# hku-mars/FAST_LIO

Hardware: NVIDIA H100
Metric: scans/sec (30k-pt scan, 1M-pt map iEKF) (higher is better)
Workload: dtype f32 geometry / f64 filter

## Files before the change

### fast_lio_b200/api.py

```python
from __future__ import annotations

import ctypes as C
import os

import numpy as np

from . import build as _build

_f32p = np.ctypeslib.ndpointer(dtype=np.float32, flags="C_CONTIGUOUS")
_f64p = np.ctypeslib.ndpointer(dtype=np.float64, flags="C_CONTIGUOUS")
_i32p = np.ctypeslib.ndpointer(dtype=np.int32, flags="C_CONTIGUOUS")
_u8p = np.ctypeslib.ndpointer(dtype=np.uint8, flags="C_CONTIGUOUS")


class PassLog(C.Structure):
    _fields_ = [("searched", C.c_int), ("valid", C.c_int), ("effct", C.c_int), ("converged", C.c_int),
                ("res_sum", C.c_double), ("HtH", C.c_double * 144), ("Hth", C.c_double * 12),
                ("x_after", C.c_double * 26)]


def _log_dict(l: PassLog) -> dict:
    return dict(searched=l.searched, valid=l.valid, effct=l.effct, converged=l.converged,
                res_sum=l.res_sum, HtH=np.array(l.HtH).reshape(12, 12).copy(),
                Hth=np.array(l.Hth).copy(), x_after=np.array(l.x_after).copy())
# ... 15 lines not shown

LIDAR_AVIA, LIDAR_VELO16, LIDAR_OUST64, LIDAR_MARSIM = 1, 2, 3, 4
TIME_SEC, TIME_MS, TIME_US, TIME_NS = 0, 1, 2, 3
CUSTOM_POINT = np.dtype({"names": ["offset_time", "x", "y", "z", "reflectivity", "tag", "line"],
                         "formats": ["<u4", "<f4", "<f4", "<f4", "u1", "u1", "u1"],
                         "offsets": [0, 4, 8, 12, 16, 17, 18], "itemsize": 20})
VELODYNE_POINT = np.dtype({"names": ["x", "y", "z", "intensity", "time", "ring"],
                           "formats": ["<f4", "<f4", "<f4", "<f4", "<f4", "<u2"],
                           "offsets": [0, 4, 8, 16, 20, 24], "itemsize": 32})
OUSTER_POINT = np.dtype({"names": ["x", "y", "z", "intensity", "t", "reflectivity", "ring", "ambient", "range"],
                         "formats": ["<f4", "<f4", "<f4", "<f4", "<u4", "<u2", "u1", "<u2", "<u4"],
                         "offsets": [0, 4, 8, 16, 20, 24, 26, 28, 32], "itemsize": 48})
POINT_XYZI = np.dtype({"names": ["x", "y", "z", "intensity"], "formats": ["<f4"] * 4, "offsets": [0, 4, 8, 16], "itemsize": 32})
DEFAULT_LAYOUT = {LIDAR_AVIA: CUSTOM_POINT, LIDAR_VELO16: VELODYNE_POINT, LIDAR_OUST64: OUSTER_POINT, LIDAR_MARSIM: POINT_XYZI}
OFFSET_FIELDS = ("x", "y", "z", "intensity", "time", "ring", "tag", "line")
_FIELD_NAMES = {LIDAR_AVIA: {"intensity": "reflectivity", "time": "offset_time"}, LIDAR_OUST64: {"time": "t"}}


def layout_offsets(dtype: np.dtype, lidar_type: int) -> list[int]:
    names = _FIELD_NAMES.get(lidar_type, {})
    fields = dtype.fields or {}
    return [int(fields[names.get(f, f)][1]) if names.get(f, f) in fields else -1 for f in OFFSET_FIELDS]


class PreprocessParams(C.Structure):
    _fields_ = [("lidar_type", C.c_int), ("n_scans", C.c_int), ("scan_rate", C.c_int), ("time_unit", C.c_int),
                ("point_filter_num", C.c_int), ("blind", C.c_double), ("point_step", C.c_int)] + \
               [("off_" + f, C.c_int) for f in OFFSET_FIELDS]


_lib = None

SYMBOLS = [
    "fl_last_error", "fl_device_count", "fl_version", "fl_host_register", "fl_host_unregister", "fl_filter_debug_prof",
    "fl_map_create", "fl_map_destroy", "fl_map_set_downsample", "fl_map_build", "fl_map_size", "fl_map_validnum",
    "fl_map_knn", "fl_map_nearest_search", "fl_map_add_points", "fl_map_delete_boxes", "fl_map_flatten", "fl_map_tree_range",
    "fl_map_rebuild", "fl_map_stats", "fl_map_add_boxes", "fl_map_box_search", "fl_map_radius_search", "fl_map_acquire_removed", "fl_map_set_cell_directory", "fl_map_dir_stats",
    "fl_map_set_deterministic", "fl_map_get_deterministic",
    "fl_map_nearest_search_device", "fl_map_range_workspace_bytes", "fl_map_box_search_device", "fl_map_radius_search_device",
    "fl_map_build_device", "fl_map_add_points_device",
    "fl_filter_create", "fl_filter_destroy", "fl_filter_set_params", "fl_filter_set_solver", "fl_filter_set_search", "fl_filter_set_fused", "fl_filter_update",
    "fl_filter_map_incremental", "fl_filter_get_nearest", "fl_filter_get_selected", "fl_filter_get_pass_logs", "fl_filter_upload_scan",
    "fl_filter_upload_state", "fl_filter_run", "fl_filter_download_state", "fl_filter_sync",
    "fl_filter_time_resident", "fl_filter_time_search_pass", "fl_filter_time_e2e", "fl_filter_gpu_launches",
    "fl_scan_create", "fl_scan_destroy", "fl_scan_upload", "fl_scan_undistort", "fl_scan_voxel_downsample", "fl_scan_download",
    "fl_filter_update_scan", "fl_localmap_create", "fl_localmap_destroy", "fl_localmap_segment", "fl_localmap_get",
    "fl_comm_unique_id", "fl_filter_comm_init", "fl_filter_set_shard", "fl_filter_p2p_handle", "fl_filter_p2p_connect",
    "fl_filter_update_device", "fl_filter_get_nearest_device", "fl_filter_get_selected_device",
    "fl_map_add_points_async", "fl_map_maintain", "fl_filter_map_incremental_device",
    "fl_scan_reserve", "fl_scan_upload_device", "fl_scan_undistort_device", "fl_scan_voxel_downsample_device",
    "fl_filter_update_scan_device", "fl_map_delete_boxes_async", "fl_localmap_segment_device",
    "fl_filter_reserve_batch", "fl_filter_batch_plan", "fl_filter_update_batch_device",
    "fl_preprocess_create", "fl_preprocess_destroy", "fl_preprocess_device", "fl_preprocess",
    "fl_scan_frame", "fl_scan_frame_device",
]


def lib_path() -> str:
    return _build.LIB


def load():
    global _lib
    if _lib is not None:
        return _lib
    if not os.path.exists(_build.LIB):
        raise FastLioError(f"{_build.LIB} is missing -- run `python -m fast_lio_b200.build` (nvcc, sm_90a); "
# ... 801 lines not shown
```

### fast_lio_b200/build.py

```python
from __future__ import annotations

import os
import shutil
import subprocess
import sys

HERE = os.path.dirname(os.path.abspath(__file__))
CSRC = os.path.join(HERE, "csrc")
LIB = os.path.join(HERE, "libfastlio_b200.so")
SOURCES = ["map.cu", "filter.cu", "scan.cu", "preprocess.cu", "capi.cu"]
HEADERS = ["common.cuh", "map.cuh", "map.h", "lie.cuh", "filter.h", "scan.h", "gj.cuh", "measure.cuh", "update.cuh", "upd_plan.h", "preprocess.h", os.path.join("..", "..", "include", "fastlio_b200.h")]

NVCC_FLAGS = [
    "-gencode", "arch=compute_90a,code=sm_90a",
    "-O3", "-std=c++17", "-lineinfo",
    "--fmad=false", "-prec-div=true", "-prec-sqrt=true",
    "-Xcompiler", "-fPIC", "-shared",
    "-Xptxas", "-v",
]


def _nvcc() -> str:
    for cand in (os.environ.get("NVCC"), "/usr/local/cuda/bin/nvcc", shutil.which("nvcc")):
        if cand and os.path.exists(cand):
            return cand
    raise RuntimeError("nvcc not found")


def needs_build() -> bool:
    if not os.path.exists(LIB):
        return True
    t = os.path.getmtime(LIB)
    deps = [os.path.join(CSRC, s) for s in SOURCES + HEADERS] + [os.path.abspath(__file__)]
    return any(os.path.getmtime(d) > t for d in deps if os.path.exists(d))


def build(force: bool = False, verbose: bool = False) -> str:
    if not force and not needs_build():
        return LIB
    tmp = LIB + ".tmp"
    cmd = [_nvcc()] + NVCC_FLAGS + ["-ccbin", "/usr/bin/g++"] + [os.path.join(CSRC, s) for s in SOURCES] + ["-o", tmp, "-ldl"]
    res = subprocess.run(cmd, capture_output=True, text=True)
    log = res.stdout + res.stderr
    with open(os.path.join(HERE, "build.log"), "w") as f:
        f.write(" ".join(cmd) + "\n" + log)
    if res.returncode != 0:
        sys.stderr.write(log)
        raise RuntimeError("nvcc failed")
    os.replace(tmp, LIB)
    if verbose:
        print(log)
    return LIB


if __name__ == "__main__":
    build(force="--force" in sys.argv, verbose=True)
```

### fast_lio_b200/csrc/capi.cu

```cuda
#include <atomic>
#include <chrono>
#include <cstring>
#include <mutex>
#include <new>

#include "../../include/fastlio_b200.h"
#include "filter.h"
#include "preprocess.h"
#include "scan.h"

namespace fl {
const char* last_error();
int nccl_unique_id(void* out128);
}

struct fl_map {
    fl::Map* impl;
    std::mutex mu;
    std::atomic<int> refs{1};
};
static void map_retain(fl_map* m) { m->refs.fetch_add(1, std::memory_order_relaxed); }
static void map_release(fl_map* m) {
    if (m->refs.fetch_sub(1, std::memory_order_acq_rel) == 1) {
        delete m->impl;
// ... 281 lines not shown
    FILTER_GUARD(f);
    if (!out3) { fl::set_last_error("fl_filter_batch_plan: null out3"); return FL_ERR_ARG; }
    return f->impl->batch_plan(nq, n_hyp, &out3[0], &out3[1], &out3[2]);
}
int fl_filter_update_batch_device(fl_filter_t* f, const float* body_xyzi_device, int nq, int n_hyp, double* x26_device, double* P_device,
                                  double R, int* status2_device, fl_pass_log_t* logs_device, void* stream) {
    FILTER_GUARD(f);
    return f->impl->update_batch_on_stream(body_xyzi_device, nq, n_hyp, x26_device, P_device, R, status2_device,
                                           reinterpret_cast<fl::PassLog*>(logs_device), static_cast<cudaStream_t>(stream));
}
int fl_filter_get_nearest_device(fl_filter_t* f, float* out_pts_device, int* out_cnt_device, int nq, void* stream) {
    FILTER_GUARD(f);
    return f->impl->get_nearest_on_stream(out_pts_device, out_cnt_device, nq, static_cast<cudaStream_t>(stream));
}
int fl_filter_get_selected_device(fl_filter_t* f, unsigned char* out_device, int nq, void* stream) {
    FILTER_GUARD(f);
    return f->impl->get_selected_on_stream(out_device, nq, static_cast<cudaStream_t>(stream));
}
int fl_filter_upload_scan(fl_filter_t* f, const float* body, int nq) { FILTER_GUARD(f); return f->impl->upload_scan(body, nq); }
int fl_filter_upload_state(fl_filter_t* f, const double* x26, const double* P, double R) {
    FILTER_GUARD(f);
    if (!x26 || !P) return FL_ERR_ARG;
    return f->impl->upload_state(x26, P, R);
}
int fl_filter_run(fl_filter_t* f) { FILTER_HOST_GUARD(f); return f->impl->run_passes(); }
int fl_filter_download_state(fl_filter_t* f, double* x26, double* P, int* n_pass) { FILTER_GUARD(f); return f->impl->download_state(x26, P, n_pass); }
int fl_filter_sync(fl_filter_t* f) { FILTER_GUARD(f); return f->impl->sync(); }
int fl_filter_debug_prof(fl_filter_t* f, long long* out16) {
    FILTER_GUARD(f);
    if (!out16) return FL_ERR_ARG;
    FL_CUDA(cudaMemcpy(out16, f->impl->ctl_device()->prof, sizeof(long long) * 16, cudaMemcpyDeviceToHost));
    for (int i = 0; i < 4; i++) out16[12 + i] = f->impl->host_ns()[i];
    return FL_OK;
}
int fl_filter_gpu_launches(fl_filter_t* f) { FILTER_GUARD(f); return f->impl->gpu_launches(); }

int fl_filter_time_resident(fl_filter_t* f, int reps, int flush_l2, float* ms_total) {
    FILTER_GUARD(f);
    if (reps < 1 || !ms_total) return FL_ERR_ARG;
    fl::Filter* F = f->impl;
    cudaStream_t st = F->stream();
    FL_CUDA(cudaSetDevice(F->map()->device()));
    const size_t flush_bytes = 256u << 20;
    if (flush_l2) FL_CHECK(f->flush.reserve(flush_bytes));
    cudaEvent_t e0, e1;
    FL_CUDA(cudaEventCreate(&e0));
    FL_CUDA(cudaEventCreate(&e1));
    float total = 0.f;
    for (int r = 0; r < reps; r++) {
        FL_CHECK(F->restore_state());
        if (flush_l2) FL_CUDA(cudaMemsetAsync(f->flush.ptr, r & 0xff, flush_bytes, st));
        FL_CHECK(F->p2p_barrier());
        FL_CUDA(cudaEventRecord(e0, st));
        int rc = F->run_passes();
        if (rc != FL_OK) { cudaEventDestroy(e0); cudaEventDestroy(e1); return rc; }
        FL_CUDA(cudaEventRecord(e1, st));
        FL_CUDA(cudaEventSynchronize(e1));
        float ms = 0.f;
        FL_CUDA(cudaEventElapsedTime(&ms, e0, e1));
        total += ms;
    }
    cudaEventDestroy(e0);
    cudaEventDestroy(e1);
    *ms_total = total;
    return FL_OK;
}
// ... 283 lines not shown
```

### fast_lio_b200/csrc/filter.cu

```cuda
#include <dlfcn.h>

#include <algorithm>
#include <chrono>
#include <cstdlib>

#include <cub/device/device_select.cuh>

#include "filter.h"
#include "gj.cuh"
#include "measure.cuh"

namespace fl {

constexpr int PSTRIDE = 96;
constexpr size_t P2P_MAIL_BYTES = sizeof(unsigned long long) * 2 * 2 * P2P_MAX_RANKS * PSTRIDE;
constexpr int SEARCH_THREADS = 256;
constexpr int SEARCH_C_THREADS = 256;
constexpr int RESID_THREADS = 256;
constexpr int MAX_LOGS = 16;

__device__ __forceinline__ void pdl_wait() { asm volatile("griddepcontrol.wait;" ::: "memory"); }
__device__ __forceinline__ void pdl_launch() { asm volatile("griddepcontrol.launch_dependents;" ::: "memory"); }

__device__ __forceinline__ int tri12(int a, int b) { return a * 12 - (a * (a - 1)) / 2 + (b - a); }
// ... 984 lines not shown
    if (nq < 0 || (nq > 0 && !body_xyzi)) { set_last_error("scan: bad arguments"); return FL_ERR_ARG; }
    FL_CUDA(cudaSetDevice(map_->device()));
    FL_CHECK(reserve(std::max(1, nq)));
    if (nq > 0) FL_CUDA(cudaMemcpyAsync(body_.ptr, body_xyzi, sizeof(float4) * (size_t)nq, cudaMemcpyHostToDevice, stream()));
    return set_scan_device(body_.as<float4>(), nq);
}

int Filter::set_shard(int q_begin, int q_end) {
    if (q_begin < 0 || q_end < q_begin) { set_last_error("set_shard: bad range"); return FL_ERR_ARG; }
    scan_.q_begin = q_begin; scan_.q_end = q_end;
    shard_set_ = true;
    return FL_OK;
}

int Filter::upload_state(const double* x26, const double* P, double R, bool snapshot) {
    FL_CUDA(cudaSetDevice(map_->device()));
    FL_CUDA(cudaStreamSynchronize(stream()));
    FilterCtl& c = *h_ctl_;
    c.iter = -1; c.t = 0; c.converge = 1; c.done = 0; c.n_pass = 0; c.error = 0; c.ticket = 0; c.gen = 0;
    c.max_iter = max_iter_;
    c.host_mirror = (mirror_ && !snapshot) ? h_ctl_ : nullptr;
    c.extrinsic_est = extrinsic_est_;
    c.R = R;
    for (int i = 0; i < NDOF; i++) c.limit[i] = limit_[i];
    memcpy(c.x, x26, sizeof(double) * XLEN);
    memcpy(c.x_prop, x26, sizeof(double) * XLEN);
    memcpy(c.P, P, sizeof(double) * NDOF * NDOF);
    memcpy(c.P_prop, P, sizeof(double) * NDOF * NDOF);
    FL_CUDA(cudaMemcpyAsync(ctl_.ptr, h_ctl_, sizeof(FilterCtl), cudaMemcpyHostToDevice, stream()));
    if (snapshot) FL_CUDA(cudaMemcpyAsync(ctl0_.ptr, ctl_.ptr, sizeof(FilterCtl), cudaMemcpyDeviceToDevice, stream()));
    return FL_OK;
}

int Filter::restore_state() {
    FL_CUDA(cudaSetDevice(map_->device()));
    FL_CUDA(cudaMemcpyAsync(ctl_.ptr, ctl0_.ptr, sizeof(FilterCtl), cudaMemcpyDeviceToDevice, stream()));
    return FL_OK;
}

template <class... KArgs, class... Args>
static cudaError_t launch_pdl_smem(void (*kernel)(KArgs...), dim3 grid, int block, size_t smem, cudaStream_t st, bool pdl, Args... args) {
    cudaLaunchConfig_t cfg;
    memset(&cfg, 0, sizeof(cfg));
    cfg.gridDim = grid; cfg.blockDim = dim3((unsigned)block); cfg.dynamicSmemBytes = smem; cfg.stream = st;
    cudaLaunchAttribute attr[1];
    attr[0].id = cudaLaunchAttributeProgrammaticStreamSerialization;
    attr[0].val.programmaticStreamSerializationAllowed = pdl ? 1 : 0;
    cfg.attrs = attr; cfg.numAttrs = 1;
    return cudaLaunchKernelEx(&cfg, kernel, KArgs(args)...);
}
template <class... KArgs, class... Args>
static cudaError_t launch_pdl(void (*kernel)(KArgs...), dim3 grid, int block, cudaStream_t st, bool pdl, Args... args) {
    return launch_pdl_smem(kernel, grid, block, 0, st, pdl, args...);
}

int Filter::complete_neighbours() {
    if (neighbours_complete_ || (scan_.q_begin <= 0 && scan_.q_end >= scan_.Q)) { neighbours_complete_ = true; return FL_OK; }
    FL_CUDA(cudaSetDevice(map_->device()));
    const int keep_b = scan_.q_begin, keep_e = scan_.q_end;
    const int ranges[2][2] = {{0, keep_b}, {keep_e, scan_.Q}};
    for (int r = 0; r < 2; r++) {
        if (ranges[r][1] <= ranges[r][0]) continue;
        scan_.q_begin = ranges[r][0]; scan_.q_end = ranges[r][1];
        UpdArgs a = upd_args(1, 0, 1);
        a.dbg = 0; a.pose_from_search = 1;
        cudaError_t e = launch_plan(plan(UR_NEIGHBOURS, scan_.q_end - scan_.q_begin), a, stream());
// ... 626 lines not shown
```

### fast_lio_b200/csrc/filter.h

```cpp
#pragma once
#include "lie.cuh"
#include "map.h"
#include "upd_plan.h"

namespace fl {

struct PassLog {
    int searched, valid, effct, converged;
    double res_sum;
    double HtH[144];
    double Hth[12];
    double x_after[XLEN];
};

struct FilterCtl {
    int iter;
    int t;
    int converge;
    int done;
    int n_pass;
    int max_iter;
    int extrinsic_est;
    int error;
    int ticket;
// ... 57 lines not shown
    int download_state(double* x26, double* P, int* n_pass);
    int sync();
    int update_on_stream(const float* d_body, int nq, double* d_x26, double* d_P, double R, int* d_status2, cudaStream_t st);
    int get_nearest_on_stream(float* d_pts, int* d_cnt, int nq, cudaStream_t st);
    int get_selected_on_stream(unsigned char* d_out, int nq, cudaStream_t st);
    int update_scan_on_stream(const float4* d_body, const int* d_n, int n_max, double* d_x26, double* d_P, double R, int* d_status2, cudaStream_t st);
    int capacity() const;
    int reserve_batch(int nq_max);
    int batch_plan(int nq, int n_hyp, int* workers, int* slots, int* waves) const;
    int update_batch_on_stream(const float* d_body, int nq, int n_hyp, double* d_x26, double* d_P, double R, int* d_status2,
                               PassLog* d_logs, cudaStream_t st);

    int map_incremental(double filter_size_map_min, int ekf_inited, int* n_to_add, int* n_no_downsample, int* added);
    int map_incremental_on_stream(double filter_size_map_min, int ekf_inited, int* d_out4, cudaStream_t st);
    int get_nearest(float* out_pts, int* out_cnt, int nq);
    int complete_neighbours();
    int get_selected(unsigned char* out, int nq);
    int get_pass_logs(PassLog* out, int cap, int* n);
    int comm_init(int nranks, int rank, const void* nccl_unique_id_128);
    int set_shard(int q_begin, int q_end);
    int p2p_local_handle(void* out64);
    int p2p_connect(int nranks, int rank, const void* handles64);
    int p2p_barrier();

    void set_fused(bool on) { fused_ = on; }
    bool fused() const { return fused_ && solver_ == 1; }
    int gpu_launches() const { return launches_; }
    const long long* host_ns() const { return host_ns_; }
    const float4* nearest_device() const { return scan_.nearest; }
    const ScanView& scan() const { return scan_; }
    cudaStream_t stream() const { return map_->stream(); }
    Map* map() const { return map_; }
    const FilterCtl* ctl_device() const { return ctl_.as<FilterCtl>(); }

private:
    int reserve(int nq);
    int update_any(const float* body_xyzi, const float4* d_body, int nq, double* x26, double* P, double R, double* solve_time_s);
    Map* map_;
    int max_points_;
    int max_iter_ = 4;
    double limit_[NDOF];
    int extrinsic_est_ = 0;
    int solver_ = 1;
    bool mirror_ = true;
    bool pdl_ = true;
    int search_occ_ = 5;
    int search_mode_ = 1;
    ScanView scan_;
    DeviceBuffer srange_;
    DeviceBuffer body_, nearest_, nearest_cnt_, selected_, normvec_, plane_, partials_, red_, ctl_, ctl0_, logs_;
    DeviceBuffer mi_world_, mi_flag_add_, mi_flag_no_, mi_list_add_, mi_list_no_, mi_tmp_, mi_counts_;
    FilterCtl* h_ctl_ = nullptr;
    cudaEvent_t ev0_ = nullptr, ev1_ = nullptr;
    int sms_ = 0, search_grid_max_ = 0, max_resid_grid_ = 0, resid_grid_ = 1;
    bool fused_ = true;
    DeviceBuffer pub_;
    unsigned launch_nonce_ = 0;
    UpdCaps upd_caps_ = {};
    int launch_update(int max_passes, int mode, int search_only) { return launch_update(max_passes, mode, search_only, stream()); }
    int launch_update(int max_passes, int mode, int search_only, cudaStream_t st);
    UpdPlan plan(UpdRoute r, int rows, int n_hyp = 0) const;
    cudaError_t launch_plan(const UpdPlan& p, const UpdArgs& a, cudaStream_t st, const int* n = nullptr, int log_stride = 0);
    StateIn state_in_args(double R) const;
    int device_form_scope(const char* what, bool update) const;
    UpdArgs upd_args(int max_passes, int mode, int search_only);
    int bind_scan(const float4* d_body, int nq);
// ... 23 lines not shown
```

### fast_lio_b200/csrc/update.cuh

```cuda
#pragma once

namespace fl {

constexpr int UPD_THREADS = 256;
constexpr int UPD_WARPS = UPD_THREADS / 32;

struct UpdArgs {
    MapView m;
    ScanView sc;
    FilterCtl* ctl;
    double* partials;
    double* red_g;
    PassLog* logs;
    P2PState* p2p;
    unsigned long long* pub;
    unsigned nonce;
    int mode;
    int max_passes;
    int search_only;
    int dbg;
    int pose_from_search;
};

struct SolverSm {
// ... 21 lines not shown
    WalkPool walks;
    unsigned pose_bits[28];
    unsigned flags;
    int abort;
};

__device__ __forceinline__ int ld_acquire(const int* p) {
    int v;
    asm volatile("ld.acquire.gpu.global.s32 %0, [%1];" : "=r"(v) : "l"(p) : "memory");
    return v;
}
__device__ __forceinline__ void st_release(int* p, int v) { asm volatile("st.release.gpu.global.s32 [%0], %1;" ::"l"(p), "r"(v) : "memory"); }
constexpr long long SPIN_LIMIT = 3000000000ll;

constexpr int PUB_WORDS = 29;
__device__ __forceinline__ unsigned pub_tag(unsigned nonce, int pass) { return (nonce << 8) | (unsigned)(pass & 0xff); }
__device__ __forceinline__ void pub_store(unsigned long long* p, unsigned tag, unsigned payload) {
    asm volatile("st.relaxed.gpu.global.u64 [%0], %1;" ::"l"(p), "l"(((unsigned long long)tag << 32) | payload) : "memory");
}
__device__ __forceinline__ unsigned long long pub_load(const unsigned long long* p) {
    unsigned long long v;
    asm volatile("ld.relaxed.gpu.global.u64 %0, [%1];" : "=l"(v) : "l"(p) : "memory");
    return v;
}
__device__ __forceinline__ void pub_publish(unsigned long long* pub, unsigned tag, const double* x, int converge, int done, int lane) {
    if (lane < 28) {
        const unsigned long long bits = (unsigned long long)__double_as_longlong(x[lane >> 1]);
        pub_store(pub + lane, tag, (lane & 1) ? (unsigned)(bits >> 32) : (unsigned)bits);
    } else if (lane == 28) {
        pub_store(pub + 28, tag, (converge ? 1u : 0u) | (done ? 2u : 0u));
    }
}


template <bool DET>
__device__ __forceinline__ void cell_scan_chunks(const MapView& m, int start, int cnt, int c0, int c1, float qx, float qy, float qz, TBestT<DET>& kb) {
    const int4* list = reinterpret_cast<const int4*>(m.dir.lists + start);
    int4 ia = make_int4(0, 0, 0, 0), ib = make_int4(0, 0, 0, 0);
    if (c0 < c1) {
        ia = __ldg(&list[2 * c0]);
        if (cnt - 8 * c0 > 4) ib = __ldg(&list[2 * c0 + 1]);
    }
#pragma unroll 1
    for (int c = c0; c < c1; c++) {
        const int n8 = cnt - 8 * c;
        float4 p0, p1, p2, p3, p4, p5, p6, p7;
        p1 = p2 = p3 = p4 = p5 = p6 = p7 = make_float4(0.f, 0.f, 0.f, 0.f);
        p0 = __ldg(&m.pts[ia.x]);
        if (n8 > 1) p1 = __ldg(&m.pts[ia.y]);
        if (n8 > 2) p2 = __ldg(&m.pts[ia.z]);
        if (n8 > 3) p3 = __ldg(&m.pts[ia.w]);
        if (n8 > 4) p4 = __ldg(&m.pts[ib.x]);
        if (n8 > 5) p5 = __ldg(&m.pts[ib.y]);
        if (n8 > 6) p6 = __ldg(&m.pts[ib.z]);
        if (n8 > 7) p7 = __ldg(&m.pts[ib.w]);
        int4 na = ia, nb = ib;
        if (c + 1 < c1) {
            na = __ldg(&list[2 * c + 2]);
            if (n8 > 12) nb = __ldg(&list[2 * c + 3]);
        }
        cell_consider(m, p0, ia.x, qx, qy, qz, kb);
        cell_consider(m, p1, ia.y, qx, qy, qz, kb);
        cell_consider(m, p2, ia.z, qx, qy, qz, kb);
        cell_consider(m, p3, ia.w, qx, qy, qz, kb);
        cell_consider(m, p4, ib.x, qx, qy, qz, kb);
        cell_consider(m, p5, ib.y, qx, qy, qz, kb);
// ... 42 lines not shown
        }
    }
    PairXch& X = *reinterpret_cast<PairXch*>(stage);
    pair_sync(warp);
    if (!owner) {
#pragma unroll
        for (int j = 0; j < KNN_K; j++) { X.d[j][lane] = kb.d[j]; X.idx[j][lane] = kb.idx[j]; }
    }
    pair_sync(warp);
    bool exact = true;
    if (owner && active) {
        exact = false;
        if (listed) {
            pair_merge(m, X, lane, kb);
            if (kb.idx[KNN_K - 1] >= 0) {
                const float g = cell_block_dist(D, qx, qy, qz, ix, iy, iz);
                exact = kb.d[KNN_K - 1] < g * g;
            }
        }
    }
    int mine_slot = -1;
    int* counter = &W.n[phase & 1];
    if (owner && active && !exact) {
        mine_slot = atomicAdd(counter, 1);
        if (mine_slot < WALK_POOL) {
            W.who[mine_slot] = (int)threadIdx.x; W.x[mine_slot] = qx; W.y[mine_slot] = qy; W.z[mine_slot] = qz;
            const bool full = kb.idx[KNN_K - 1] >= 0;
#pragma unroll
            for (int j = 0; j < KNN_K; j++) { W.rd[mine_slot][j] = full ? kb.d[j] : INFINITY; W.ri[mine_slot][j] = full ? kb.idx[j] : -1; }
        }
    }
    __syncthreads();
    const int total = *counter, n = min(total, WALK_POOL);
    if (threadIdx.x == 0) W.n[(phase + 1) & 1] = 0;
    phase++;
    for (int i = warp; i < n; i += nwarps) {
        KBestT<DET> w;
        w.init();
        if (lane < KNN_K) { w.d = W.rd[i][lane]; w.idx = W.ri[i][lane]; }
        w.w = __shfl_sync(FULL, w.d, KNN_K - 1);
        w.n = w.w < INFINITY ? KNN_K : 0;
        knn_query_from(m, W.x[i], W.y[i], W.z[i], w, lane);
        __syncwarp();
        if (lane < KNN_K) { W.rd[i][lane] = w.d; W.ri[i][lane] = w.idx; }
    }
    unsigned todo = __ballot_sync(FULL, mine_slot >= WALK_POOL);
    while (todo) {
        const int src = __ffs(todo) - 1;
        todo &= todo - 1;
        KBestT<DET> w;
        knn_query(m, __shfl_sync(FULL, qx, src), __shfl_sync(FULL, qy, src), __shfl_sync(FULL, qz, src), w, lane);
#pragma unroll
        for (int j = 0; j < KNN_K; j++) {
            const float dj = __shfl_sync(FULL, w.d, j);
            const int ij = __shfl_sync(FULL, w.idx, j);
            if (lane == src) { kb.d[j] = dj; kb.idx[j] = ij; }
        }
    }
    __syncthreads();
    if (mine_slot >= 0 && mine_slot < WALK_POOL) {
#pragma unroll
        for (int j = 0; j < KNN_K; j++) { kb.d[j] = W.rd[mine_slot][j]; kb.idx[j] = W.ri[mine_slot][j]; }
    }
    if (threadIdx.x == 0 && total && m.dir.cap && m.dir.n_walked) atomicAdd(m.dir.n_walked, total);
}

template <bool EXTR, int PAIR, bool DET>
__device__ __forceinline__ bool measure_fused(const MapView& m, const ScanView& sc, int q, bool active, const PoseS& s, bool searched,
                                              bool search_only, WalkPool& walks, int& phase, double* stage, double* h, double& z, float& absres) {
    float4 pb = make_float4(0.f, 0.f, 0.f, 0.f);
    float wx = 0.f, wy = 0.f, wz = 0.f;
    D3 p_this = d3(0.0, 0.0, 0.0);
    if (active) {
        pb = __ldg(&sc.body[q]);
        p_this = body_to_world(s, pb, wx, wy, wz);
    }
    bool sel = false;
    float pabcd[4] = {0.f, 0.f, 0.f, 0.f};
    if (searched) {
        TBestT<DET> kb;
        if constexpr (PAIR == 1) {
            knn_block(m, active, wx, wy, wz, kb, walks, phase);
        } else {
            knn_block_pair(m, active, wx, wy, wz, kb, walks, phase, stage);
            if (threadIdx.x >= UPD_THREADS) return false;
        }
        if (active) {
            float4 p[KNN_K];
            const int cnt = knn_fetch(m, kb, p);
#pragma unroll
            for (int j = 0; j < KNN_K; j++) sc.nearest[(size_t)q * KNN_K + j] = p[j];
            sc.nearest_cnt[q] = cnt;
// ... 505 lines not shown
    float4 plane[UPD_THREADS];
    double srange[UPD_THREADS];
    unsigned char sel[UPD_THREADS];
};
constexpr int WAVE_EPOCH = 32;
__device__ __forceinline__ unsigned row_tag(unsigned epoch, int pass) { return pub_tag(epoch, pass + 1); }
__device__ __forceinline__ unsigned long long globaltimer() {
    unsigned long long t;
    asm volatile("mov.u64 %0, %%globaltimer;" : "=l"(t));
    return t;
}
__device__ __forceinline__ ulonglong2 row_load(const unsigned long long* p) {
    ulonglong2 v;
    asm volatile("ld.relaxed.gpu.global.v2.u64 {%0, %1}, [%2];" : "=l"(v.x), "=l"(v.y) : "l"(p) : "memory");
    return v;
}
__device__ __forceinline__ bool row_current(ulonglong2 v, unsigned tag) { return (unsigned)(v.x >> 32) == tag && (unsigned)(v.y >> 32) == tag; }
__device__ __forceinline__ double row_value(ulonglong2 v) { return __longlong_as_double((long long)((v.y << 32) | (v.x & 0xffffffffull))); }

template <bool EXTR, bool DET>
__device__ __forceinline__ bool measure_wave(const MapView& m, const ScanView& sc, int q, bool active, const PoseS& s, bool searched,
                                             bool search_only, WalkPool& walks, int& phase, double* stage, WavePoint& pt, double* h,
                                             double& z, float& absres) {
    const int i = threadIdx.x & (UPD_THREADS - 1);
    float4 pb = make_float4(0.f, 0.f, 0.f, 0.f);
    float wx = 0.f, wy = 0.f, wz = 0.f;
    D3 p_this = d3(0.0, 0.0, 0.0);
    if (active) {
        pb = pt.body[i];
        p_this = body_to_world(s, pb, wx, wy, wz);
    }
    bool sel = false;
    float pabcd[4] = {0.f, 0.f, 0.f, 0.f};
    if (searched) {
        TBestT<DET> kb;
        knn_block_pair(m, active, wx, wy, wz, kb, walks, phase, stage);
        if (threadIdx.x >= UPD_THREADS) return false;
        if (active) {
            float4 p[KNN_K];
            const int cnt = knn_fetch(m, kb, p);
#pragma unroll
            for (int j = 0; j < KNN_K; j++) sc.nearest[(size_t)q * KNN_K + j] = p[j];
            sc.nearest_cnt[q] = cnt;
            sel = knn_gate(cnt, kb.d[KNN_K - 1]);
            if (search_only) { sc.selected[q] = sel ? 1 : 0; return false; }
            if (sel) {
                float pn[KNN_K][3];
#pragma unroll
                for (int j = 0; j < KNN_K; j++) { pn[j][0] = p[j].x; pn[j][1] = p[j].y; pn[j][2] = p[j].z; }
                sel = esti_plane_dev(pabcd, pn, 0.1f);
                if (sel) { const float4 pl = make_float4(pabcd[0], pabcd[1], pabcd[2], pabcd[3]); sc.plane[q] = pl; pt.plane[i] = pl; }
            }
        }
    } else if (active) {
        sel = pt.sel[i] != 0;
        if (sel) { const float4 pl = pt.plane[i]; pabcd[0] = pl.x; pabcd[1] = pl.y; pabcd[2] = pl.z; pabcd[3] = pl.w; }
    }
    bool contrib = false;
    if (active && sel) {
        const float pd2 = plane_residual(pabcd, wx, wy, wz);
        const double srange = pt.srange[i];
        if (searched) sc.srange[q] = srange;
        float score;
        if (score_gate(pd2, srange, score)) {
            contrib = true;
            absres = fabsf(pd2);
            jacobian_row_at<EXTR>(s, pb, p_this, make_float4(pabcd[0], pabcd[1], pabcd[2], pd2), h, z);
        }
    }
    if (active) { sc.selected[q] = contrib ? 1 : 0; pt.sel[i] = contrib ? 1 : 0; }
    return contrib;
}

constexpr int GATHER_ROWS = 8;
__device__ void sol_gather(SolverSm& S, FilterCtl* ctl, const unsigned long long* __restrict__ rows, int nwork, unsigned tag) {
    const int tid = threadIdx.x, lane = tid & 31, warp = tid >> 5;
    double a0 = 0.0, a1 = 0.0, a2 = 0.0;
    bool late = false;
    const long long t0 = clock64();
    for (int b = warp; b < nwork; b += GATHER_ROWS * UPD_WARPS) {
        const unsigned long long* base = rows + (size_t)b * PSTRIDE * 2 + 2 * lane;
        ulonglong2 v[GATHER_ROWS][3];
#pragma unroll
        for (int k = 0; k < GATHER_ROWS; k++) {
#pragma unroll
            for (int j = 0; j < 3; j++) v[k][j] = make_ulonglong2(0ull, 0ull);
            if (b + k * UPD_WARPS < nwork) {
#pragma unroll
                for (int j = 0; j < 3; j++) v[k][j] = row_load(base + (size_t)k * UPD_WARPS * PSTRIDE * 2 + 64 * j);
            }
        }
        while (true) {
            bool stale = false;
#pragma unroll
            for (int k = 0; k < GATHER_ROWS; k++) {
#pragma unroll
                for (int j = 0; j < 3; j++) stale |= b + k * UPD_WARPS < nwork && !row_current(v[k][j], tag);
            }
            if (!stale) break;
            if (clock64() - t0 > SPIN_LIMIT) { late = true; break; }
#pragma unroll
            for (int k = 0; k < GATHER_ROWS; k++) {
#pragma unroll
                for (int j = 0; j < 3; j++) {
                    if (b + k * UPD_WARPS < nwork && !row_current(v[k][j], tag)) v[k][j] = row_load(base + (size_t)k * UPD_WARPS * PSTRIDE * 2 + 64 * j);
                }
            }
        }
#pragma unroll
        for (int k = 0; k < GATHER_ROWS; k++) {
            if (b + k * UPD_WARPS < nwork) { a0 += row_value(v[k][0]); a1 += row_value(v[k][1]); a2 += row_value(v[k][2]); }
        }
        if (late) break;
    }
    S.wred[warp][lane] = a0; S.wred[warp][lane + 32] = a1; S.wred[warp][lane + 64] = a2;
    if (late) S.late = 2;
    sol_sync();
    if (tid == 0) ctl->prof[9] = clock64();
    if (tid < PSTRIDE) {
        double v = 0.0;
#pragma unroll
        for (int w = 0; w < UPD_WARPS; w++) v += S.wred[w][tid];
        S.red[tid] = v;
        if (tid < 78) {
            int a = 0, rem = tid;
            while (rem >= 12 - a) { rem -= 12 - a; a++; }
            const int b = a + rem;
            S.HTH[a * 12 + b] = v; S.HTH[b * 12 + a] = v;
        }
    }
    sol_sync();
    if (tid == 128) ctl->prof[11] = (long long)globaltimer();
}

template <bool EXTR, bool DET = false>
__device__ __forceinline__ void update_wave_body(const UpdArgs& a, unsigned long long* __restrict__ rows, const int q1) {
    static_assert(sizeof(PairXch) <= sizeof(double) * WorkerSm<EXTR>::STAGE, "the partner's list fits the owner warp's stage slice");
    __shared__ __align__(16) unsigned char smem_raw[sizeof(SolverSm) > sizeof(WorkerSm<EXTR>) ? sizeof(SolverSm) : sizeof(WorkerSm<EXTR>)];
    extern __shared__ __align__(16) unsigned char wave_dyn[];
    __shared__ volatile int solver_ended;
    FilterCtl* ctl = a.ctl;
    const int tid = threadIdx.x, lane = tid & 31, warp = tid >> 5;
    const int nwork = (int)gridDim.x - 1;
    pdl_wait();
    pdl_launch();
    const unsigned epoch = (unsigned)__ldcg(a.pub + WAVE_EPOCH) + 1u;
    if (blockIdx.x > 0) {
        WorkerSm<EXTR>& Wk = *reinterpret_cast<WorkerSm<EXTR>*>(smem_raw);
        WavePoint& pt = *reinterpret_cast<WavePoint*>(wave_dyn);
        const int wb = (int)blockIdx.x - 1;
        const int i = tid & (UPD_THREADS - 1), q = a.sc.q_begin + wb * UPD_THREADS + i;
        const bool active = q < q1, owner = tid < UPD_THREADS;
        if (tid == 0) { Wk.abort = 0; Wk.walks.n[0] = Wk.walks.n[1] = 0; }
        int walk_phase = 0;
        double* stage = Wk.stage[warp & (UPD_WARPS - 1)];
        for (int p = 0; p < a.max_passes; p++) {
            PoseS s;
            bool searched;
            if (p == 0) {
                const bool done = __ldcg(&ctl->done) != 0;
                searched = __ldcg(&ctl->converge) != 0 || a.search_only;
                s = load_pose(a.pose_from_search ? ctl->x_search : ctl->x);
                if (owner && active) {
                    const float4 pb = __ldg(&a.sc.body[q]);
                    pt.body[i] = pb;
                    pt.srange[i] = sqrt(norm3(d3(pb.x, pb.y, pb.z)));
                    if (!searched) {
                        pt.sel[i] = a.sc.selected[q];
                        if (pt.sel[i]) { pt.plane[i] = a.sc.plane[q]; pt.srange[i] = a.sc.srange[q]; }
                    }
                }
                __syncthreads();
                if (done && !a.search_only) return;
            } else {
                const unsigned tag = pub_tag(a.nonce, p);
                if (warp == 0 && lane < PUB_WORDS) {
                    unsigned long long w = pub_load(a.pub + lane);
                    const long long t0 = clock64();
                    while ((unsigned)(w >> 32) != tag) {
                        if (clock64() - t0 > SPIN_LIMIT) { Wk.abort = 1; atomicExch(&ctl->error, 3); break; }
                        w = pub_load(a.pub + lane);
                    }
                    if (lane < 28) Wk.pose_bits[lane] = (unsigned)w; else Wk.flags = (unsigned)w;
                }
                __syncthreads();
                if (Wk.abort) return;
                if (Wk.flags & 2u) {
                    if (tid == 0) atomicMax(reinterpret_cast<unsigned long long*>(&ctl->prof[3]), globaltimer());
                    return;
                }
                searched = (Wk.flags & 1u) != 0;
                double x14[14];
#pragma unroll
                for (int k = 0; k < 14; k++) x14[k] = __longlong_as_double((long long)(((unsigned long long)Wk.pose_bits[2 * k + 1] << 32) | Wk.pose_bits[2 * k]));
                s.pos = d3(x14[X_POS], x14[X_POS + 1], x14[X_POS + 2]);
                s.rot.x = x14[X_ROT]; s.rot.y = x14[X_ROT + 1]; s.rot.z = x14[X_ROT + 2]; s.rot.w = x14[X_ROT + 3];
                s.offR.x = x14[X_OFFR]; s.offR.y = x14[X_OFFR + 1]; s.offR.z = x14[X_OFFR + 2]; s.offR.w = x14[X_OFFR + 3];
                s.offT = d3(x14[X_OFFT], x14[X_OFFT + 1], x14[X_OFFT + 2]);
            }
            double acc[3] = {0.0, 0.0, 0.0};
            double h[12]; double z = 0.0; float ar = 0.f;
            bool contrib = false;
            if (owner || searched)
                contrib = measure_wave<EXTR, DET>(a.m, a.sc, q, active, s, searched, a.search_only != 0, Wk.walks, walk_phase, stage, pt, h, z, ar);
            if (owner && !a.search_only) warp_accumulate<EXTR>(contrib, h, z, ar, acc, lane, stage);
            if (a.search_only) return;
            if (owner) {
#pragma unroll
                for (int j = 0; j < 3; j++) Wk.wred[warp][lane + 32 * j] = acc[j];
            }
            __syncthreads();
            if (tid < PSTRIDE) {
                double v = 0.0;
#pragma unroll
                for (int w = 0; w < UPD_WARPS; w++) v += Wk.wred[w][tid];
                const unsigned long long bits = (unsigned long long)__double_as_longlong(v);
                unsigned long long* dst = rows + ((size_t)wb * PSTRIDE + tid) * 2;
                const unsigned tag = row_tag(epoch, p);
                pub_store(dst, tag, (unsigned)bits);
                pub_store(dst + 1, tag, (unsigned)(bits >> 32));
            }
        }
        return;
    }
    if (a.search_only) return;
    if (tid == 0) solver_ended = 0;
    __syncthreads();
    if (tid >= UPD_THREADS) {
        if (tid == UPD_THREADS) {
            for (int p = 1; p <= a.max_passes; p++) {
                const unsigned tag = pub_tag(a.nonce, p);
                unsigned long long w;
                while ((unsigned)((w = pub_load(a.pub + 28)) >> 32) != tag) if (solver_ended) return;
                ctl->prof[2] = (long long)globaltimer();
                if (w & 2u) return;
            }
        }
        return;
    }
    SolverSm& S = *reinterpret_cast<SolverSm*>(smem_raw);
    sol_load(S, ctl);
    for (int p = 0; p < a.max_passes && !S.done; p++) {
        if (tid == 0) ctl->prof[0] = clock64();
        if (S.converge && tid < XLEN) ctl->x_search[tid] = S.x[tid];
        sol_prepare(S);
        if (tid == 0) ctl->prof[8] = clock64();
        sol_gather(S, ctl, rows, nwork, row_tag(epoch, p));
        if (tid == 0) ctl->prof[1] = clock64();
        sol_pass<EXTR>(S, ctl, a.logs, a.pub, pub_tag(a.nonce, p + 1));
        if (tid == 0) ctl->prof[7] = clock64();
    }
    if (tid == 0) {
        ctl->error = S.error | ctl->error; ctl->ticket = 0;
        a.pub[WAVE_EPOCH] = epoch;
        solver_ended = 1;
    }
    sol_sync();
    mirror_copy(ctl, UPD_THREADS);
}

template <bool EXTR>
__global__ void __launch_bounds__(2 * UPD_THREADS, 1) k_update_wave(UpdArgs a, unsigned long long* rows) {
    update_wave_body<EXTR>(a, rows, a.sc.q_end);
}
template <bool EXTR>
__global__ void __launch_bounds__(2 * UPD_THREADS, 1) k_update_n_wave(UpdArgs a, const int* __restrict__ n, unsigned long long* rows) {
    update_wave_body<EXTR>(a, rows, min(*n, a.sc.q_end));
}

template <bool EXTR, int PAIR>
__global__ void __launch_bounds__(UPD_THREADS * PAIR, 3 - PAIR) k_update_det(UpdArgs a) {
    update_body<EXTR, PAIR, true>(a, a.sc.q_end);
}
template <bool EXTR, int PAIR>
__global__ void __launch_bounds__(UPD_THREADS * PAIR, 3 - PAIR) k_update_n_det(UpdArgs a, const int* __restrict__ n) {
    update_body<EXTR, PAIR, true>(a, min(*n, a.sc.q_end));
}
template <bool EXTR>
__global__ void __launch_bounds__(UPD_THREADS, 2) k_update_batch_det(UpdArgs a, int log_stride) {
    update_batch_body<EXTR, true>(a, log_stride);
// ... 12 lines not shown
```

### include/fastlio_b200.h

```cpp
#ifndef FASTLIO_B200_H
#define FASTLIO_B200_H

#ifdef __cplusplus
extern "C" {
#endif

#define FL_OK 0
#define FL_ERR_CUDA (-1)
#define FL_ERR_ARG (-2)
#define FL_ERR_NCCL (-3)
#define FL_ERR_STATE (-4)
#define FL_ERR_CAPACITY (-5)

typedef struct fl_map fl_map_t;
typedef struct fl_filter fl_filter_t;

typedef struct fl_pass_log {
    int searched, valid, effct, converged;
    double res_sum;
    double HtH[144];
    double Hth[12];
    double x_after[26];
} fl_pass_log_t;

// ... 36 lines not shown
int fl_map_delete_boxes_async(fl_map_t* m, const float* boxes6_device, const int* nb_device, int nb_max, int* status2_device,
                              void* stream);
int fl_map_maintain(fl_map_t* m, int* layout_changed);
int fl_map_tree_range(fl_map_t* m, float* box6);
int fl_map_rebuild(fl_map_t* m);
int fl_map_stats(fl_map_t* m, int* out4);
int fl_map_set_cell_directory(fl_map_t* m, int on, float cell_size);
int fl_map_set_deterministic(fl_map_t* m, int on);
int fl_map_get_deterministic(fl_map_t* m, int* on);
int fl_map_dir_stats(fl_map_t* m, int* out6);

int fl_filter_create(fl_filter_t** out, fl_map_t* map, int max_points);
int fl_filter_destroy(fl_filter_t* f);
int fl_filter_set_params(fl_filter_t* f, int max_iter, const double* limit23, int extrinsic_est_en);
int fl_filter_set_solver(fl_filter_t* f, int mode);
int fl_filter_set_search(fl_filter_t* f, int mode);
int fl_filter_set_fused(fl_filter_t* f, int on);
int fl_filter_update(fl_filter_t* f, const float* body_xyzi, int nq, double* x26, double* P, double R, double* solve_time_s);
int fl_filter_map_incremental(fl_filter_t* f, double filter_size_map_min, int flg_EKF_inited, int* out3);
int fl_filter_get_nearest(fl_filter_t* f, float* out_pts, int* out_cnt, int nq);
int fl_filter_get_selected(fl_filter_t* f, unsigned char* out, int nq);
int fl_filter_get_pass_logs(fl_filter_t* f, fl_pass_log_t* out, int cap);
int fl_filter_upload_scan(fl_filter_t* f, const float* body_xyzi, int nq);
int fl_filter_upload_state(fl_filter_t* f, const double* x26, const double* P, double R);
int fl_filter_run(fl_filter_t* f);
int fl_filter_download_state(fl_filter_t* f, double* x26, double* P, int* n_pass);
int fl_filter_sync(fl_filter_t* f);
int fl_filter_time_resident(fl_filter_t* f, int reps, int flush_l2, float* ms_total);
int fl_filter_time_e2e(fl_filter_t* f, const float* body_xyzi, int nq, const double* x26, const double* P, double R, int reps,
                       double* seconds, double* x26_out, double* P_out);
int fl_filter_time_search_pass(fl_filter_t* f, int reps, int flush_l2, float* ms_total);
int fl_filter_gpu_launches(fl_filter_t* f);
int fl_filter_debug_prof(fl_filter_t* f, long long* out16);

int fl_filter_update_device(fl_filter_t* f, const float* body_xyzi_device, int nq, double* x26_device, double* P_device, double R,
                            int* status2_device, void* stream);
int fl_filter_get_nearest_device(fl_filter_t* f, float* out_pts_device, int* out_cnt_device, int nq, void* stream);
int fl_filter_get_selected_device(fl_filter_t* f, unsigned char* out_device, int nq, void* stream);
int fl_filter_map_incremental_device(fl_filter_t* f, double filter_size_map_min, int flg_EKF_inited, int* out4_device, void* stream);

int fl_filter_reserve_batch(fl_filter_t* f, int nq_max);
int fl_filter_batch_plan(fl_filter_t* f, int nq, int n_hyp, int* out3);
int fl_filter_update_batch_device(fl_filter_t* f, const float* body_xyzi_device, int nq, int n_hyp, double* x26_device,
                                  double* P_device, double R, int* status2_device, fl_pass_log_t* logs_device, void* stream);

typedef struct fl_scan fl_scan_t;
int fl_scan_create(fl_scan_t** out, fl_map_t* map);
int fl_scan_destroy(fl_scan_t* s);
int fl_scan_upload(fl_scan_t* s, const float* xyzi, const float* offset_ms, int n);
int fl_scan_undistort(fl_scan_t* s, const double* imu_pose22, int n_pose, const double* x26_end);
int fl_scan_voxel_downsample(fl_scan_t* s, float leaf_size);
int fl_scan_download(fl_scan_t* s, int which, float* out_xyzi, int cap);
int fl_filter_update_scan(fl_filter_t* f, fl_scan_t* s, double* x26, double* P, double R, double* solve_time_s);

int fl_scan_reserve(fl_scan_t* s, int n_max, int n_pose_max);
int fl_scan_upload_device(fl_scan_t* s, const float* xyzi_device, const float* offset_ms_device, const int* n_device, int n_max,
                          void* stream);
int fl_scan_undistort_device(fl_scan_t* s, const double* imu_pose22_device, const int* n_pose_device, int n_pose_max,
                             const double* x26_end_device, void* stream);
int fl_scan_voxel_downsample_device(fl_scan_t* s, float leaf_size, int* n_out_device, void* stream);
int fl_filter_update_scan_device(fl_filter_t* f, fl_scan_t* s, double* x26_device, double* P_device, double R, int* status2_device,
                                 void* stream);

#define FL_FRAME_LIDAR 0
#define FL_FRAME_IMU 1
#define FL_FRAME_WORLD 2
// ... 44 lines not shown
```

Measured before the change: 12380.

## Move row gathering to helper warps of block 0 and add timeline probe

The per-pass reduction of published rows now runs on the extra warps of block 0 (threads at or above UPD_THREADS) instead of the solver warps. The helper warps arrive on a named barrier once their partial sums are in shared memory, and the solver warps sync on that barrier before summing. This lets the gathering overlap with the solver's preparation work, and the helpers then wait for the next pass's publish. A compile-time-gated device timeline instrumentation and its API entry point are also added; they are off by default. The risk is barrier or ordering mistakes between the helper and solver warps, and reuse of dynamic shared memory in block 0.

```diff
diff --git a/fast_lio_b200/api.py b/fast_lio_b200/api.py
--- a/fast_lio_b200/api.py
+++ b/fast_lio_b200/api.py
@@ -71,7 +71,7 @@
 _lib = None
 
 SYMBOLS = [
-    "fl_last_error", "fl_device_count", "fl_version", "fl_host_register", "fl_host_unregister", "fl_filter_debug_prof",
+    "fl_last_error", "fl_device_count", "fl_version", "fl_host_register", "fl_host_unregister", "fl_filter_debug_prof", "fl_filter_debug_timeline",
     "fl_map_create", "fl_map_destroy", "fl_map_set_downsample", "fl_map_build", "fl_map_size", "fl_map_validnum",
     "fl_map_knn", "fl_map_nearest_search", "fl_map_add_points", "fl_map_delete_boxes", "fl_map_flatten", "fl_map_tree_range",
     "fl_map_rebuild", "fl_map_stats", "fl_map_add_boxes", "fl_map_box_search", "fl_map_radius_search", "fl_map_acquire_removed", "fl_map_set_cell_directory", "fl_map_dir_stats",
diff --git a/fast_lio_b200/build.py b/fast_lio_b200/build.py
--- a/fast_lio_b200/build.py
+++ b/fast_lio_b200/build.py
@@ -35,19 +35,20 @@
     return any(os.path.getmtime(d) > t for d in deps if os.path.exists(d))
 
 
-def build(force: bool = False, verbose: bool = False) -> str:
-    if not force and not needs_build():
+def build(force: bool = False, verbose: bool = False, out: str = "", defines: tuple = ()) -> str:
+    lib = os.path.abspath(out) if out else LIB
+    if not out and not force and not needs_build():
         return LIB
-    tmp = LIB + ".tmp"
-    cmd = [_nvcc()] + NVCC_FLAGS + ["-ccbin", "/usr/bin/g++"] + [os.path.join(CSRC, s) for s in SOURCES] + ["-o", tmp, "-ldl"]
+    tmp = lib + ".tmp"
+    cmd = [_nvcc()] + NVCC_FLAGS + [f"-D{d}" for d in defines] + ["-ccbin", "/usr/bin/g++"] + [os.path.join(CSRC, s) for s in SOURCES] + ["-o", tmp, "-ldl"]
     res = subprocess.run(cmd, capture_output=True, text=True)
     log = res.stdout + res.stderr
-    with open(os.path.join(HERE, "build.log"), "w") as f:
+    with open(os.path.join(os.path.dirname(lib), "build.log"), "w") as f:
         f.write(" ".join(cmd) + "\n" + log)
     if res.returncode != 0:
         sys.stderr.write(log)
         raise RuntimeError("nvcc failed")
-    os.replace(tmp, LIB)
+    os.replace(tmp, lib)
     if verbose:
         print(log)
     return LIB
diff --git a/fast_lio_b200/csrc/capi.cu b/fast_lio_b200/csrc/capi.cu
--- a/fast_lio_b200/csrc/capi.cu
+++ b/fast_lio_b200/csrc/capi.cu
@@ -337,6 +337,10 @@
     FL_CUDA(cudaMemcpy(out16, f->impl->ctl_device()->prof, sizeof(long long) * 16, cudaMemcpyDeviceToHost));
     for (int i = 0; i < 4; i++) out16[12 + i] = f->impl->host_ns()[i];
     return FL_OK;
+}
+int fl_filter_debug_timeline(fl_filter_t* f, long long* stamps, int n_stamps, int* cells, int n_cells) {
+    FILTER_GUARD(f);
+    return f->impl->debug_timeline(stamps, n_stamps, cells, n_cells);
 }
 int fl_filter_gpu_launches(fl_filter_t* f) { FILTER_GUARD(f); return f->impl->gpu_launches(); }
 
diff --git a/fast_lio_b200/csrc/filter.cu b/fast_lio_b200/csrc/filter.cu
--- a/fast_lio_b200/csrc/filter.cu
+++ b/fast_lio_b200/csrc/filter.cu
@@ -1040,6 +1040,27 @@
     return FL_OK;
 }
 
+int Filter::debug_timeline(long long* stamps, int n_stamps, int* cells, int n_cells) {
+#ifdef FL_UPDATE_TIMELINE
+    if (n_stamps < 0 || n_cells < 0 || (n_stamps && !stamps) || (n_cells && !cells)) return FL_ERR_ARG;
+    FL_CUDA(cudaSetDevice(map_->device()));
+    FL_CUDA(cudaStreamSynchronize(stream()));
+    void* tl = nullptr;
+    void* tc = nullptr;
+    FL_CUDA(cudaGetSymbolAddress(&tl, g_update_timeline));
+    FL_CUDA(cudaGetSymbolAddress(&tc, g_update_cells));
+    const size_t bt = sizeof(g_update_timeline), bc = sizeof(g_update_cells);
+    FL_CUDA(cudaMemcpy(stamps, tl, std::min(bt, sizeof(long long) * (size_t)n_stamps), cudaMemcpyDeviceToHost));
+    FL_CUDA(cudaMemcpy(cells, tc, std::min(bc, sizeof(int) * (size_t)n_cells), cudaMemcpyDeviceToHost));
+    FL_CUDA(cudaMemset(tl, 0, bt));
+    FL_CUDA(cudaMemset(tc, 0xff, bc));
+    return FL_OK;
+#else
+    (void)stamps; (void)n_stamps; (void)cells; (void)n_cells;
+    return FL_ERR_STATE;
+#endif
+}
+
 int Filter::restore_state() {
     FL_CUDA(cudaSetDevice(map_->device()));
     FL_CUDA(cudaMemcpyAsync(ctl_.ptr, ctl0_.ptr, sizeof(FilterCtl), cudaMemcpyDeviceToDevice, stream()));
diff --git a/fast_lio_b200/csrc/filter.h b/fast_lio_b200/csrc/filter.h
--- a/fast_lio_b200/csrc/filter.h
+++ b/fast_lio_b200/csrc/filter.h
@@ -113,6 +113,7 @@
     cudaStream_t stream() const { return map_->stream(); }
     Map* map() const { return map_; }
     const FilterCtl* ctl_device() const { return ctl_.as<FilterCtl>(); }
+    int debug_timeline(long long* stamps, int n_stamps, int* cells, int n_cells);
 
 private:
     int reserve(int nq);
diff --git a/fast_lio_b200/csrc/update.cuh b/fast_lio_b200/csrc/update.cuh
--- a/fast_lio_b200/csrc/update.cuh
+++ b/fast_lio_b200/csrc/update.cuh
@@ -77,6 +77,29 @@
     }
 }
 
+#ifdef FL_UPDATE_TIMELINE
+constexpr int TL_PASSES = 8, TL_BLOCKS = 192, TL_SLOTS = 8, TL_POINTS = 1 << 15;
+enum { TL_POSE = 0, TL_SEARCH, TL_WALKS, TL_NWALK, TL_FIT, TL_ROW, TL_SEARCHED, TL_PASS };
+enum { TL_SUMMED = 0, TL_PUB };
+__device__ long long g_update_timeline[TL_PASSES][TL_BLOCKS][TL_SLOTS];
+__device__ int4 g_update_cells[TL_PASSES][TL_POINTS];
+__device__ __forceinline__ unsigned long long tl_now() {
+    unsigned long long t;
+    asm volatile("mov.u64 %0, %%globaltimer;" : "=l"(t));
+    return t;
+}
+__device__ __forceinline__ unsigned long long* tl_block() {
+    __shared__ unsigned long long s[TL_SLOTS];
+    return s;
+}
+__device__ __forceinline__ void tl_stamp_last(int slot) {
+    if (threadIdx.x == blockDim.x - 1) tl_block()[slot] = tl_now();
+}
+#define TL(...) __VA_ARGS__
+#else
+#define TL(...)
+#endif
+
 
 template <bool DET>
 __device__ __forceinline__ void cell_scan_chunks(const MapView& m, int start, int cnt, int c0, int c1, float qx, float qy, float qz, TBestT<DET>& kb) {
@@ -185,6 +208,7 @@
     }
     __syncthreads();
     const int total = *counter, n = min(total, WALK_POOL);
+    TL(tl_stamp_last(TL_SEARCH); if (threadIdx.x == blockDim.x - 1) tl_block()[TL_NWALK] = total;)
     if (threadIdx.x == 0) W.n[(phase + 1) & 1] = 0;
     phase++;
     for (int i = warp; i < n; i += nwarps) {
@@ -211,6 +235,7 @@
         }
     }
     __syncthreads();
+    TL(tl_stamp_last(TL_WALKS);)
     if (mine_slot >= 0 && mine_slot < WALK_POOL) {
 #pragma unroll
         for (int j = 0; j < KNN_K; j++) { kb.d[j] = W.rd[mine_slot][j]; kb.idx[j] = W.ri[mine_slot][j]; }
@@ -782,6 +807,12 @@
     }
     bool sel = false;
     float pabcd[4] = {0.f, 0.f, 0.f, 0.f};
+    TL(if (searched && active && threadIdx.x < UPD_THREADS && q < TL_POINTS && m.dir.cap != 0u) {
+        const int ix = cell_coord(wx, m.dir.inv_cell), iy = cell_coord(wy, m.dir.inv_cell), iz = cell_coord(wz, m.dir.inv_cell);
+        int start, cnt;
+        if (cell_list(m.dir, cell_key(ix, iy, iz), start, cnt) <= 0) cnt = -1;
+        g_update_cells[tl_block()[TL_PASS]][q] = make_int4(ix, iy, iz, cnt);
+    })
     if (searched) {
         TBestT<DET> kb;
         knn_block_pair(m, active, wx, wy, wz, kb, walks, phase, stage);
@@ -823,8 +854,12 @@
 }
 
 constexpr int GATHER_ROWS = 8;
-__device__ void sol_gather(SolverSm& S, FilterCtl* ctl, const unsigned long long* __restrict__ rows, int nwork, unsigned tag) {
-    const int tid = threadIdx.x, lane = tid & 31, warp = tid >> 5;
+struct WaveSums {
+    double wred[UPD_WARPS][PSTRIDE];
+    int late[UPD_WARPS];
+};
+__device__ __forceinline__ void sol_gather_rows(WaveSums& G, const unsigned long long* __restrict__ rows, int nwork, unsigned tag) {
+    const int lane = threadIdx.x & 31, warp = (threadIdx.x >> 5) - UPD_WARPS;
     double a0 = 0.0, a1 = 0.0, a2 = 0.0;
     bool late = false;
     const long long t0 = clock64();
@@ -863,14 +898,19 @@
         }
         if (late) break;
     }
-    S.wred[warp][lane] = a0; S.wred[warp][lane + 32] = a1; S.wred[warp][lane + 64] = a2;
-    if (late) S.late = 2;
-    sol_sync();
+    G.wred[warp][lane] = a0; G.wred[warp][lane + 32] = a1; G.wred[warp][lane + 64] = a2;
+    late = __any_sync(FULL, late);
+    if (lane == 0) G.late[warp] = late ? 1 : 0;
+    asm volatile("bar.arrive 3, 512;" ::: "memory");
+}
+__device__ void sol_sum_rows(SolverSm& S, FilterCtl* ctl, const WaveSums& G) {
+    const int tid = threadIdx.x;
+    asm volatile("bar.sync 3, 512;" ::: "memory");
     if (tid == 0) ctl->prof[9] = clock64();
     if (tid < PSTRIDE) {
         double v = 0.0;
 #pragma unroll
-        for (int w = 0; w < UPD_WARPS; w++) v += S.wred[w][tid];
+        for (int w = 0; w < UPD_WARPS; w++) v += G.wred[w][tid];
         S.red[tid] = v;
         if (tid < 78) {
             int a = 0, rem = tid;
@@ -879,8 +919,10 @@
             S.HTH[a * 12 + b] = v; S.HTH[b * 12 + a] = v;
         }
     }
+    if (tid < UPD_WARPS && G.late[tid]) S.late = 2;
     sol_sync();
     if (tid == 128) ctl->prof[11] = (long long)globaltimer();
+    TL(if (tid == 128 && S.n_pass < TL_PASSES) g_update_timeline[S.n_pass][0][TL_SUMMED] = ctl->prof[11];)
 }
 
 template <bool EXTR, bool DET = false>
@@ -907,6 +949,7 @@
         for (int p = 0; p < a.max_passes; p++) {
             PoseS s;
             bool searched;
+            TL(if (tid == 0) tl_block()[TL_PASS] = min(p, TL_PASSES - 1);)
             if (p == 0) {
                 const bool done = __ldcg(&ctl->done) != 0;
                 searched = __ldcg(&ctl->converge) != 0 || a.search_only;
@@ -948,11 +991,13 @@
                 s.offR.x = x14[X_OFFR]; s.offR.y = x14[X_OFFR + 1]; s.offR.z = x14[X_OFFR + 2]; s.offR.w = x14[X_OFFR + 3];
                 s.offT = d3(x14[X_OFFT], x14[X_OFFT + 1], x14[X_OFFT + 2]);
             }
+            TL(tl_stamp_last(TL_POSE); if (tid == blockDim.x - 1) tl_block()[TL_SEARCHED] = searched ? 1 : 0;)
             double acc[3] = {0.0, 0.0, 0.0};
             double h[12]; double z = 0.0; float ar = 0.f;
             bool contrib = false;
             if (owner || searched)
                 contrib = measure_wave<EXTR, DET>(a.m, a.sc, q, active, s, searched, a.search_only != 0, Wk.walks, walk_phase, stage, pt, h, z, ar);
+            TL(if (owner && lane == 0) atomicMax(&tl_block()[TL_FIT], tl_now());)
             if (owner && !a.search_only) warp_accumulate<EXTR>(contrib, h, z, ar, acc, lane, stage);
             if (a.search_only) return;
             if (owner) {
@@ -970,21 +1015,35 @@
                 pub_store(dst, tag, (unsigned)bits);
                 pub_store(dst + 1, tag, (unsigned)(bits >> 32));
             }
+            TL(if (tid == 0) {
+                unsigned long long* st = tl_block();
+                st[TL_ROW] = tl_now();
+                if (p < TL_PASSES && blockIdx.x < TL_BLOCKS) {
+                    for (int k = 0; k < TL_SLOTS; k++) g_update_timeline[p][blockIdx.x][k] = (long long)st[k];
+                }
+                st[TL_SEARCH] = st[TL_WALKS] = st[TL_NWALK] = st[TL_FIT] = 0;
+            })
         }
         return;
     }
     if (a.search_only) return;
+    static_assert(sizeof(WaveSums) <= sizeof(WavePoint), "the gathered sums fit block 0's dynamic shared memory");
+    WaveSums& G = *reinterpret_cast<WaveSums*>(wave_dyn);
     if (tid == 0) solver_ended = 0;
     __syncthreads();
     if (tid >= UPD_THREADS) {
-        if (tid == UPD_THREADS) {
-            for (int p = 1; p <= a.max_passes; p++) {
-                const unsigned tag = pub_tag(a.nonce, p);
-                unsigned long long w;
-                while ((unsigned)((w = pub_load(a.pub + 28)) >> 32) != tag) if (solver_ended) return;
+        if (__ldcg(&ctl->done) != 0) return;
+        for (int p = 0; p < a.max_passes; p++) {
+            sol_gather_rows(G, rows, nwork, row_tag(epoch, p));
+            if (p + 1 >= a.max_passes) return;
+            const unsigned tag = pub_tag(a.nonce, p + 1);
+            unsigned long long w;
+            while ((unsigned)((w = pub_load(a.pub + 28)) >> 32) != tag) if (solver_ended) return;
+            if (tid == UPD_THREADS) {
                 ctl->prof[2] = (long long)globaltimer();
-                if (w & 2u) return;
-            }
+                TL(if (p < TL_PASSES) g_update_timeline[p][0][TL_PUB] = ctl->prof[2];)
+            }
+            if (w & 2u) return;
         }
         return;
     }
@@ -995,7 +1054,7 @@
         if (S.converge && tid < XLEN) ctl->x_search[tid] = S.x[tid];
         sol_prepare(S);
         if (tid == 0) ctl->prof[8] = clock64();
-        sol_gather(S, ctl, rows, nwork, row_tag(epoch, p));
+        sol_sum_rows(S, ctl, G);
         if (tid == 0) ctl->prof[1] = clock64();
         sol_pass<EXTR>(S, ctl, a.logs, a.pub, pub_tag(a.nonce, p + 1));
         if (tid == 0) ctl->prof[7] = clock64();
diff --git a/include/fastlio_b200.h b/include/fastlio_b200.h
--- a/include/fastlio_b200.h
+++ b/include/fastlio_b200.h
@@ -92,6 +92,7 @@
 int fl_filter_time_search_pass(fl_filter_t* f, int reps, int flush_l2, float* ms_total);
 int fl_filter_gpu_launches(fl_filter_t* f);
 int fl_filter_debug_prof(fl_filter_t* f, long long* out16);
+int fl_filter_debug_timeline(fl_filter_t* f, long long* stamps, int n_stamps, int* cells, int n_cells);
 
 int fl_filter_update_device(fl_filter_t* f, const float* body_xyzi_device, int nq, double* x26_device, double* P_device, double R,
                             int* status2_device, void* stream);
```

After: 12600 (median of 6 runs). +1.8%, better.
